# caomuqing/neptune

Measured on AMD Instinct MI355X. Metric: backend_replans_per_sec, higher is better.
Workload: dtype f64; 1 GPU; 64 agents + 20 static obstacles, K=8, 128 seeded scenes in flight per GPU per step (seeds 0..127 over 1 GPU); the handle's default solve path: verified line presolve 4 m, polish on; agents=64, obstacles=20, scenes_per_gpu=128, scenes_in_flight=128, scene_groups=1

## Files before the change

### include/neptune_backend_debug.h

```cpp
#ifndef NEPTUNE_BACKEND_DEBUG_H
#define NEPTUNE_BACKEND_DEBUG_H

#include "neptune_backend.h"

#ifdef __cplusplus
extern "C" {
#endif

int nep_backend_debug_time_sequence(nep_backend_t* h, const nep_pwp* init, int32_t n_obst, const int32_t* hull_off,
                                    const double* hull_xy, const int32_t* h0_off, const double* h0_xy, const nep_ent_view* ent,
                                    double t_start, double dc, int32_t n_iter, double* us_out, double* us_optimize_out);

int nep_backend_debug_set_lines(nep_backend_t* h, int32_t n_lines, const int32_t* seg,
                                const double* nd);
int nep_backend_debug_get_lines(nep_backend_t* h, int32_t cap, int32_t* seg, double* nd,
                                int32_t* n_out);

int nep_debug_regroup_records(const nep_traj_rec* d_src, nep_traj_rec* d_dst, int32_t world, int32_t n_scenes,
                              int32_t n_local, void* stream);

int nep_batch_debug_redo_count(nep_batch_t* h, int32_t* by_reason);
int nep_batch_debug_redo_list(nep_batch_t* h, int32_t* slots_out, int32_t cap);

int64_t nep_batch_line_bucket_bytes(nep_batch_t* h);
// ... 16 lines not shown

int nep_batch_debug_conflicts(nep_batch_t* h, int32_t scene, uint8_t* conflict_out);
int nep_batch_debug_conflicts_prev(nep_batch_t* h, int32_t scene, uint8_t* conflict_out);

int nep_batch_kernel_time(nep_batch_t* h, int32_t which, double* avg_ms, int32_t* n_launch);
int nep_batch_enable_timing(nep_batch_t* h, int32_t on);
int nep_batch_reset_timing(nep_batch_t* h);

enum {
  NEP_PATH_BOX_KERNEL = 1,
  NEP_PATH_HULLS_GROUPED = 2,
  NEP_PATH_FUSED_BOXES = 4,
  NEP_PATH_FUSED_ORDER = 8,
  NEP_PATH_ORDERED_QP = 16,
  NEP_PATH_PRESOLVE_KERNEL = 32,
  NEP_PATH_REDO_PASS = 64
};
int nep_batch_debug_launch_path(nep_batch_t* h, int32_t* bits);
int nep_batch_debug_boxes(nep_batch_t* h, int32_t scene, double* out, int32_t cap);
int nep_batch_debug_order_keys(nep_batch_t* h, int32_t* keys, int32_t cap);

int nep_batch_debug_hulls(nep_batch_t* h, int32_t scene, double* hull_xy, int32_t* hull_nv);
int nep_batch_debug_lines(nep_batch_t* h, int32_t slot, int32_t cap, int32_t* seg, double* nd,
                          int32_t* n_out);

int nep_batch_debug_phase_cycles(nep_batch_t* h, int32_t slot, int64_t* out16);

int nep_batch_fe_search_us(nep_batch_t* h, float* us, int32_t cap);

int nep_batch_set_fe_ent_fast_caps(nep_batch_t* h, int32_t list_cap, int32_t add_cap, int32_t bend_cap);

// ... 10 lines not shown
```

### neptune_amd/abi.py

```python
import ctypes as C

import numpy as np

NEP_MAX_POL = 8
NEP_TRAJ_MAX_SEG = 16
NEP_HULL_MAX_V = 16
NEP_HULL_MAX_CP = 16
NEP_MAX_BEND = 8
NEP_STATE_DOUBLES = 12

NEP_OK, NEP_RELAXED, NEP_FAILED = 0, 1, 2
NEP_SKIPPED = 3
NEP_FE_SKIPPED = 4


class nep_pwp(C.Structure):
    _fields_ = [("n_seg", C.c_int32), ("_pad", C.c_int32),
                ("times", C.c_double * (NEP_TRAJ_MAX_SEG + 1)),
                ("coeff", ((C.c_double * 4) * NEP_TRAJ_MAX_SEG) * 3)]


class nep_traj_rec(C.Structure):
    _fields_ = [("id", C.c_int32), ("is_agent", C.c_int32), ("n_bend", C.c_int32),
                ("valid", C.c_int32),
                ("bbox", C.c_double * 3), ("pos", C.c_double * 3),
                ("bend", (C.c_double * 2) * NEP_MAX_BEND),
                ("pwp", nep_pwp)]

# ... 187 lines not shown
```

### neptune_amd/backend.py

```python
import ctypes as C

import numpy as np

from . import abi
from ._lib import BackendError, check, lib


def _csr(polys):
    off = np.zeros(len(polys) + 1, dtype=np.int32)
    for k, p in enumerate(polys):
        off[k + 1] = off[k] + len(p)
    xy = (np.concatenate([np.asarray(p, dtype=np.float64).reshape(-1, 2) for p in polys])
          if len(polys) and off[-1] > 0 else np.zeros((0, 2)))
    return off, np.ascontiguousarray(xy, dtype=np.float64)


def make_pwp(times, coeff):
    p = abi.nep_pwp()
    K = coeff.shape[1]
    p.n_seg = K
    for i in range(K + 1):
        p.times[i] = float(times[i])
    arr = np.ctypeslib.as_array(p.coeff)
    arr[:, :K, :] = coeff
# ... 426 lines not shown
    def qp_kernel_name(self):
        return "qp_reg_kernel" if lib().nep_batch_qp_placement(self._h) == 1 else "qp_kernel"

    def set_hull_kernel(self, mode=0):
        check(lib().nep_batch_set_hull_kernel(self._h, int(mode)))

    def set_launch_order(self, enable=True):
        check(lib().nep_batch_set_launch_order(self._h, 1 if enable else 0))

    def launch_order(self):
        out = np.zeros(self.n_scenes * self.n_local, dtype=np.int32); n = C.c_int32(0)
        check(lib().nep_batch_debug_launch_order(self._h, abi.iptr(out), len(out), C.byref(n)))
        return out[:n.value].copy() if n.value else None

    LAUNCH_PATH = (("box_kernel", 1), ("grouped_hulls", 2), ("fused_boxes", 4), ("fused_order", 8), ("ordered_qp", 16),
                   ("presolve_kernel", 32), ("redo_pass", 64))

    def debug_launch_path(self):
        b = C.c_int32(0)
        check(lib().nep_batch_debug_launch_path(self._h, C.byref(b)))
        return {name: bool(b.value & bit) for name, bit in self.LAUNCH_PATH}

    def debug_boxes(self, scene=0):
        out = np.zeros((self.N + self.n_static, self.par.num_pol, 4))
        check(lib().nep_batch_debug_boxes(self._h, int(scene), abi.dptr(out), out.size))
        return out

    def debug_order_keys(self):
        out = np.zeros(self.slots, dtype=np.int32)
        check(lib().nep_batch_debug_order_keys(self._h, abi.iptr(out), len(out)))
        return out
# ... 129 lines not shown
```

### neptune_amd/csrc/backend.hip

```cpp
#include <hip/hip_runtime.h>

#include <atomic>
#include <chrono>
#include <cmath>
#include <cstdio>
#include <cstdlib>
#include <cstring>
#include <memory>
#include <string>
#include <vector>

#include "nep_device.h"
#include "audit_common.h"
#include "mission_common.h"
#include "../../include/neptune_plan.h"
#include "../../include/neptune_entangle.h"

using namespace nep;

namespace nep { DebugGlobals g_debug; }

namespace {

thread_local std::string g_err;
// ... 343 lines not shown
  }
  hipEvent_t next_event() {
    if (ev_used == ev.size()) { hipEvent_t e; hipEventCreate(&e); ev.push_back(e); }
    return ev[ev_used++];
  }
  int run(const nep_traj_rec* d_recs, int n_rec, ProblemSet& ps, hipStream_t st, int phases = 3) {
    const int slots = n_scenes * sp.n_local;
    SampleSched sc{d_sched_n.p, d_sched_seg.p, d_sched_dt.p};
    const bool geo = (phases & 1) != 0, qp = (phases & 2) != 0;
    if (timing) hipEventRecord(next_event(), st);
    const bool fused_boxes = d_recs && geo && ps.skip_box != nullptr && !ps.lines_override && static_boxes_ok && ps.hull_pb <= 0
                             && n_rec == sp.num_agents && sp.n_hull == sp.num_agents && hulls_grouped(sp, n_scenes, n_rec);
    const bool want_order = qp && lpt && have_history && slots > 1024 && d_order_key.n >= (size_t)slots && d_order.n >= (size_t)slots;
    const bool fused_order = fused_boxes && want_order;
    if (fused_order) { ps.order = d_order.p; ps.order_key = d_order_key.p; }
    if (geo) last_path = 0; else last_path &= NEP_PATH_BOX_KERNEL | NEP_PATH_HULLS_GROUPED | NEP_PATH_FUSED_BOXES | NEP_PATH_FUSED_ORDER;
    if (d_recs && geo) launch_hulls(d_recs, n_scenes, n_rec, ps.guess, sp, ps, st, fused_boxes);
    if (d_recs && geo && hulls_grouped(sp, n_scenes, n_rec)) last_path |= NEP_PATH_HULLS_GROUPED;
    if (fused_boxes) last_path |= NEP_PATH_FUSED_BOXES;
    if (fused_order) last_path |= NEP_PATH_FUSED_ORDER;
    if (timing) hipEventRecord(next_event(), st);
    if (ps.lines_override) { ps.skip_box = nullptr; ps.line_skip = nullptr; ps.redo_list = nullptr; ps.redo_count = nullptr; }
    if (scratch_chunks > 0 && ps.scratch_chunks == 0) {
      scratch_full = true;
      HIPCHK(hipStreamSynchronize(st));
      if (int e = size_row_scratch()) return e;
      ps.row_scratch = d_row_scratch.p;
    }
    const bool skip = ps.skip_box != nullptr;
    if (!ps.lines_override && geo) {
      if (skip && !fused_boxes) { launch_boxes(n_scenes, sp, ps, st); last_path |= NEP_PATH_BOX_KERNEL; }
      launch_separator(slots, sp, ps, st);
    }
// ... 1378 lines not shown
  return 0;
}
int nep_batch_debug_set_option(nep_batch_t* h, const char* name, int32_t value) { if (!h) return fail(NEP_E_ARG, "null handle"); return engine_option(h->eng, name, value); }
int nep_backend_debug_set_option(nep_backend_t* h, const char* name, int32_t value) { if (!h) return fail(NEP_E_ARG, "null handle"); return engine_option(h->eng, name, value); }
int nep_debug_set_global_option(const char* name, int32_t value) {
  if (!name) return fail(NEP_E_ARG, "null option name");
  const std::string n(name);
  if (n == "fe_three") g_debug.fe_three = value != 0;
  else if (n == "fe_xcd") g_debug.fe_xcd = value;
  else if (n == "polish_grid") { if (value < 1) return fail(NEP_E_ARG, "polish_grid >= 1"); g_debug.polish_grid = value; }
  else return fail(NEP_E_ARG, "unknown global debug option: " + n);
  return 0;
}

int nep_batch_set_hull_kernel(nep_batch_t* h, int32_t mode) {
  if (!h || mode < 0 || mode > 2) return fail(NEP_E_ARG, "mode: 0 automatic, 1 one hull per wave, 2 eight hulls per wave");
  h->eng.sp.hull_mode = mode;
  return 0;
}

int nep_batch_set_max_runtime(nep_batch_t* h, double seconds) {
  if (!h || !(seconds >= 0.0)) return fail(NEP_E_ARG, "bad arguments");
  h->eng.sp.time_limit_ticks = seconds > 0 ? (long long)(seconds * h->eng.clock_hz) : 0;
  return 0;
}

namespace {
int set_line_cull(Engine* E, double radius) {
  if (!E || !(radius >= 0.0)) return fail(NEP_E_ARG, "bad arguments");
  E->sp.cull_radius = radius; E->cull_user_set = true;
  return 0;
// ... 206 lines not shown
```

### neptune_amd/csrc/geom_kernels.hip

```cpp
#include <hip/hip_runtime.h>

#include <cstdlib>
#include <cstring>

#include "nep_device.h"
#include "../../include/neptune_frontend.h"
#include "ent_device.h"

namespace nep {

__constant__ double cAPosInv[4][4] = {
    {-0.03203276669713047, -0.09273093424558249, 0.3420572455666699, 1.1023313949144335},
    {-0.05111494245568798, -0.046272612998418894, 0.5458234872124772, 1.0979806946005568},
    {-0.07454781852812224, 0.203951949894552, 0.796048050105448, 1.0745478185281223},
    {1.0, 1.0, 0.9999999999999996, 0.9999999999999993}};

#define SEP_MIN_GAP 1e-7
#define NEP_INF (__builtin_huge_val())

__device__ __forceinline__ double cross3(double ox, double oy, double ax, double ay, double bx, double by) {
  return (ax - ox) * (by - oy) - (ay - oy) * (bx - ox);
}
__device__ __forceinline__ bool lex_less(double ax, double ay, double bx, double by) {
  return ax < bx || (ax == bx && ay < by);
// ... 165 lines not shown
      const bool m_lt = (kx[r] < ox) | ((kx[r] == ox) & (ky[r] < oy));
      const bool take = want_min ? o_lt : m_lt;
      kx[r] = take ? ox : kx[r]; ky[r] = take ? oy : ky[r];
    }
  }
}
template <int J, int K_, int JJ> __device__ __forceinline__ void grp_bitonic_merge(double (&kx)[J], double (&ky)[J], int sub) {
  grp_bitonic_step<J, K_, JJ>(kx, ky, sub);
  if constexpr (JJ > 1) grp_bitonic_merge<J, K_, JJ / 2>(kx, ky, sub);
}
template <int J, int K_> __device__ __forceinline__ void grp_bitonic(double (&kx)[J], double (&ky)[J], int sub) {
  if constexpr (K_ > 2) grp_bitonic<J, K_ / 2>(kx, ky, sub);
  grp_bitonic_merge<J, K_, K_ / 2>(kx, ky, sub);
}

template <int J>
__device__ __forceinline__ int group_hull(int n, const double (&px)[J], const double (&py)[J], double* sxy, int g, int sub,
                                          bool write, double* __restrict__ out_xy, int cap) {
  constexpr int kGrpPts = J;
  __syncthreads();
  {
    double kx[J], ky[J];
#pragma unroll
    for (int j = 0; j < J; j++) { const bool in = sub + 8 * j < n; kx[j] = in ? px[j] : NEP_INF; ky[j] = in ? py[j] : NEP_INF; }
    grp_bitonic<J, 8 * J>(kx, ky, sub);
#pragma unroll
    for (int r = 0; r < J; r++) { const int e = sub * J + r; if (e < n) { sxy[2 * e] = kx[r]; sxy[2 * e + 1] = ky[r]; } }
  }
  __syncthreads();
  double ux[kGrpPts], uy[kGrpPts]; int pos[kGrpPts]; bool keep[kGrpPts];
  int m = 0;
#pragma unroll
  for (int j = 0; j < kGrpPts; j++) {
    const int p = sub + 8 * j;
    ux[j] = 0; uy[j] = 0; keep[j] = false;
    if (p < n) { ux[j] = sxy[2 * p]; uy[j] = sxy[2 * p + 1]; keep[j] = p == 0 || ux[j] != sxy[2 * p - 2] || uy[j] != sxy[2 * p - 1]; }
    const unsigned bits = (unsigned)(__ballot(keep[j]) >> (8 * g)) & 0xffu;
    pos[j] = m + __popc(bits & ((1u << sub) - 1u));
    m += __popc(bits);
  }
  __syncthreads();
#pragma unroll
  for (int j = 0; j < kGrpPts; j++) { if (keep[j]) { sxy[2 * pos[j]] = ux[j]; sxy[2 * pos[j] + 1] = uy[j]; } }
  __syncthreads();
  unsigned long long mask = 0;
  if (sub < 2 && m >= 2) {
    const bool lower = sub == 0;
    int kc = 0;
    int i1 = 0, i2 = 0;
    double ax = 0, ay = 0, bx = 0, by = 0;
    for (int i = 0; i < m; i++) {
      const double2 c = *(const double2*)(sxy + 2 * (lower ? i : m - 1 - i));
      const double x = c.x, y = c.y;
      while (kc >= 2 && cross3(ax, ay, bx, by, x, y) <= 0.0) {
        mask &= ~(1ull << i1);
        kc--; bx = ax; by = ay; i1 = i2;
        if (kc >= 2) {
          i2 = 63 - __clzll((long long)(mask & ((1ull << i2) - 1ull)));
          const double2 a = *(const double2*)(sxy + 2 * (lower ? i2 : m - 1 - i2));
          ax = a.x; ay = a.y;
        }
      }
      mask |= 1ull << i; kc++;
      ax = bx; ay = by; bx = x; by = y;
      i2 = i1; i1 = i;
    }
  }
  const unsigned long long L = __shfl(mask, 8 * g), U = __shfl(mask, 8 * g + 1);
  const int kl = __popcll(L), ku = __popcll(U);
  const int k = m >= 2 ? kl + ku - 2 : m;
  if (write) {
    if (m == 1) { if (sub == 0 && cap > 0) { out_xy[0] = sxy[0]; out_xy[1] = sxy[1]; } }
    else if (m >= 2) {
#pragma unroll
      for (int j = 0; j < kGrpPts; j++) {
        const int p = sub + 8 * j;
        if (p < m) {
          const double x = sxy[2 * p], y = sxy[2 * p + 1];
          if ((L >> p) & 1ull) { const int o = __popcll(L & ((1ull << p) - 1ull)); if (o < cap) { out_xy[2 * o] = x; out_xy[2 * o + 1] = y; } }
          const int iu = m - 1 - p;
          if (((U >> iu) & 1ull) && p != 0 && p != m - 1) {
            const int o = kl + __popcll(U & ((1ull << iu) - 1ull)) - 1;
            if (o < cap) { out_xy[2 * o] = x; out_xy[2 * o + 1] = y; }
          }
        }
      }
    }
  }
  return k;
}

__global__ __launch_bounds__(64) void hull_group_kernel(const nep_traj_rec* __restrict__ recs, int n_rec_per_scene,
                                                        const double* __restrict__ ts0, long ts_scene_stride,
                                                        int num_pol, double T_span, double drone_radius,
                                                        double* __restrict__ hull_xy, int* __restrict__ hull_nv,
                                                        double* __restrict__ hull0_xy, int* __restrict__ hull0_nv,
                                                        double* __restrict__ bend_xy, int* __restrict__ bend_n, int* __restrict__ flags,
                                                        double* __restrict__ box_out, int box_per_scene, int* __restrict__ zero4,
                                                        int n_traj, int ord_n, const int* __restrict__ ord_key, int* __restrict__ ord_out, int* __restrict__ ord_zero4) {
  __shared__ __attribute__((aligned(16))) double s_sxy[8][kGrpSxy];
  __shared__ double s_cpx[8][kHullCP], s_cpy[8][kHullCP];
  double* stimes = &s_sxy[7][0];
  static_assert(NEP_TRAJ_MAX_SEG + 2 <= kGrpSxy, "the knot vector borrows a group's point area");
  const int lane = threadIdx.x, g = lane >> 3, sub = lane & 7;
  if (ord_n > 0 && blockIdx.x == 0) {
    if (ord_zero4 && lane < 4) ord_zero4[lane] = 0;
    int* hist = (int*)&s_sxy[0][0];
    int* tot = hist + 64 * 16;
    for (int i = lane; i < 64 * 16; i += 64) hist[i] = 0;
    __syncthreads();
    const int su = lane & 15;
    for (int i0 = 0; i0 < ord_n; i0 += 1024) {
      int kk[16];
#pragma unroll
      for (int u = 0; u < 16; u++) { const int i = i0 + 64 * u + lane; kk[u] = i < ord_n ? ord_key[i] : 0; }
#pragma unroll
      for (int u = 0; u < 16; u++) { const int i = i0 + 64 * u + lane; if (i < ord_n) atomicAdd(&hist[(63 - (kk[u] & 63)) * 16 + su], 1); }
    }
    __syncthreads();
    { int o = 0; for (int u = 0; u < 16; u++) { const int c = hist[lane * 16 + u]; hist[lane * 16 + u] = o; o += c; } tot[lane] = o; }
    __syncthreads();
    if (lane == 0) { int o = 0; for (int b = 0; b < 64; b++) { const int c = tot[b]; tot[b] = o; o += c; } }
    __syncthreads();
    for (int i0 = 0; i0 < ord_n; i0 += 1024) {
      int kk[16];
#pragma unroll
      for (int u = 0; u < 16; u++) { const int i = i0 + 64 * u + lane; kk[u] = i < ord_n ? ord_key[i] : 0; }
#pragma unroll
      for (int u = 0; u < 16; u++) { const int i = i0 + 64 * u + lane; if (i < ord_n) { const int b = 63 - (kk[u] & 63); ord_out[tot[b] + atomicAdd(&hist[b * 16 + su], 1)] = i; } }
    }
    return;
  }
  const int jt = (int)blockIdx.x - (ord_n > 0 ? 1 : 0);
  const int scene = jt / n_rec_per_scene;
  const nep_traj_rec* r = recs + jt;
  if (lane == 0 && bend_n) {
    int nb = r->n_bend; if (nb > kBend) nb = kBend; if (nb < 0) nb = 0;
    bend_n[jt] = (r->valid && r->is_agent) ? nb : 0;
    for (int b = 0; b < nb; b++) { bend_xy[((long)jt * kBend + b) * 2] = r->bend[b][0]; bend_xy[((long)jt * kBend + b) * 2 + 1] = r->bend[b][1]; }
  }
  const bool act = g < num_pol;
  const long out = (long)jt * num_pol + g;
  if (zero4 && jt == 0 && lane < 4) zero4[lane] = 0;
  double* box = box_out ? box_out + (((long)scene * box_per_scene + (jt - scene * n_rec_per_scene)) * num_pol + g) * 4 : nullptr;
  if (!(r->valid && r->is_agent) || r->pwp.n_seg <= 0) {
    if (act && sub == 0) { hull_nv[out] = 0; if (hull0_nv) hull0_nv[out] = 0; if (box) { box[0] = NEP_INF; box[1] = -NEP_INF; box[2] = NEP_INF; box[3] = -NEP_INF; } }
    return;
  }
  const double ts = *(const double*)((const char*)ts0 + (long)scene * ts_scene_stride);
  const double t0 = ts + g * T_span, t1 = ts + (g + 1) * T_span;
  const int n = r->pwp.n_seg;
  if (lane <= n) stimes[lane] = r->pwp.times[lane];
  __syncthreads();
  int first = -1, last = -1;
  for (int k = 0; k <= n; k++) { const double tk = stimes[k]; first += tk < t0 ? 1 : 0; last += tk <= t1 ? 1 : 0; }
  if (first < 0) first = 0; if (first > n - 1) first = n - 1;
  if (last < 0) last = 0; if (last > n - 1) last = n - 1;
  int nseg = last - first + 1; if (nseg < 0) nseg = 0;
  if (nseg > kHullCP / 4) { nseg = kHullCP / 4; if (act && sub == 0 && flags) atomicOr(flags, NEP_FLAG_HULL_OVERFLOW); }
  if (!act) nseg = 0;
  const int np0 = 4 * nseg;
  double* cpx = s_cpx[g]; double* cpy = s_cpy[g];
  for (int v = sub; v < 2 * np0; v += 8) {
    const int sl = v >> 3, k = (v >> 1) & 3, ax = v & 1;
    const int s = first + sl;
    double _t;
    if (s != last) _t = stimes[s + 1] - stimes[s];
    else if (t1 > stimes[s + 1]) _t = stimes[s + 1] - stimes[s];
    else _t = t1 - stimes[s];
    if (_t > T_span) _t = T_span; else if (_t < 0) _t = 0;
    const double c0 = _t * _t * _t, c1 = _t * _t, c2 = _t, c3 = 1.0;
    const double* P = r->pwp.coeff[ax][s];
    const double val = (((P[0] * c0) * cAPosInv[0][k] + (P[1] * c1) * cAPosInv[1][k]) + (P[2] * c2) * cAPosInv[2][k]) + (P[3] * c3) * cAPosInv[3][k];
    if (ax == 0) cpx[sl * 4 + k] = val; else cpy[sl * 4 + k] = val;
  }
  __syncthreads();
  const double dx = r->bbox[0] / 2.0 + drone_radius, dy = r->bbox[1] / 2.0 + drone_radius;
  const bool inflate = !(sqrt(dx * dx + dy * dy) < 1e-6);
  const int np = inflate ? 4 * np0 : np0;
  double px[kGrpPts], py[kGrpPts];
#pragma unroll
  for (int j = 0; j < kGrpPts; j++) {
    const int p = sub + 8 * j;
    px[j] = 0; py[j] = 0;
    if (p < np) {
      if (inflate) {
        const int c = p >> 2, q = p & 3;
        const double x = cpx[c], y = cpy[c];
        px[j] = (q < 2) ? x + dx : x - dx;
        py[j] = (q == 0 || q == 3) ? y + dy : y - dy;
      } else { px[j] = cpx[p]; py[j] = cpy[p]; }
    }
  }
  if (box) {
    double x0 = NEP_INF, x1 = -NEP_INF, y0 = NEP_INF, y1 = -NEP_INF;
#pragma unroll
    for (int j = 0; j < 2; j++) { const int p = sub + 8 * j; if (p < np0) { const double x = cpx[p], y = cpy[p]; x0 = fmin(x0, x); x1 = fmax(x1, x); y0 = fmin(y0, y); y1 = fmax(y1, y); } }
    auto shl4 = [](double v) { return __hiloint2double(__builtin_amdgcn_mov_dpp(__double2hiint(v), 0x104, 0xf, 0xf, false), __builtin_amdgcn_mov_dpp(__double2loint(v), 0x104, 0xf, 0xf, false)); };
    x0 = fmin(x0, shl4(x0)); x1 = fmax(x1, shl4(x1)); y0 = fmin(y0, shl4(y0)); y1 = fmax(y1, shl4(y1));
    x0 = fmin(x0, grp_xor<2>(x0)); x1 = fmax(x1, grp_xor<2>(x1)); y0 = fmin(y0, grp_xor<2>(y0)); y1 = fmax(y1, grp_xor<2>(y1));
    x0 = fmin(x0, grp_xor<1>(x0)); x1 = fmax(x1, grp_xor<1>(x1)); y0 = fmin(y0, grp_xor<1>(y0)); y1 = fmax(y1, grp_xor<1>(y1));
    if (act && sub == 0) {
      if (np0 <= 0) { box[0] = NEP_INF; box[1] = -NEP_INF; box[2] = NEP_INF; box[3] = -NEP_INF; }
      else if (inflate) { box[0] = x0 - dx; box[1] = x1 + dx; box[2] = y0 - dy; box[3] = y1 + dy; }
      else { box[0] = x0; box[1] = x1; box[2] = y0; box[3] = y1; }
    }
  }
  int k = group_hull<kGrpPts>(np, px, py, s_sxy[g], g, sub, act, hull_xy + out * kHullV * 2, kHullV);
  if (k > kHullV) { k = kHullV; if (act && sub == 0 && flags) atomicOr(flags, NEP_FLAG_HULL_OVERFLOW); }
  if (act && sub == 0) hull_nv[out] = k;
  if (hull0_nv) {
    double qx[2], qy[2];
#pragma unroll
    for (int j = 0; j < 2; j++) { const int p = sub + 8 * j; qx[j] = p < np0 ? cpx[p] : 0; qy[j] = p < np0 ? cpy[p] : 0; }
    int k0 = group_hull<2>(np0, qx, qy, s_sxy[g], g, sub, act, hull0_xy + out * 2, 1);
    if (k0 > kHullV) k0 = kHullV;
    if (act && sub == 0) hull0_nv[out] = k0;
  }
}

bool hulls_grouped(const SceneParams& sp, int n_scenes, int n_rec) {
  return sp.num_pol <= 8 && (sp.hull_mode ? sp.hull_mode == 2 : (long)n_scenes * n_rec > 2048);
}
void launch_hulls(const nep_traj_rec* recs, int n_scenes, int n_rec, const nep_guess* guess,
                  const SceneParams& sp, const ProblemSet& ps, hipStream_t st, bool boxes) {
  launch_hulls_ts(recs, n_scenes, n_rec, &guess->t_start, (long)sizeof(nep_guess), sp, ps, st, boxes);
}
void launch_hulls_ts(const nep_traj_rec* recs, int n_scenes, int n_rec, const double* ts0, long ts_slot_stride,
                     const SceneParams& sp, const ProblemSet& ps, hipStream_t st, bool boxes) {
  int blocks = n_scenes * n_rec * sp.num_pol;
  if (blocks <= 0) return;
  const bool need0 = sp.ent_enabled != 0;
  const bool grouped = sp.hull_mode ? sp.hull_mode == 2 : (long)n_scenes * n_rec > 2048;
  if (sp.num_pol <= 8 && grouped) {
    const bool ord = boxes && ps.order != nullptr && ps.order_key != nullptr;
    hipLaunchKernelGGL(hull_group_kernel, dim3(n_scenes * n_rec + (ord ? 1 : 0)), dim3(64), 0, st, recs, n_rec, ts0, ts_slot_stride * sp.n_local,
                       sp.num_pol, sp.T_span, sp.drone_radius, ps.hull_xy, ps.hull_nv, need0 ? ps.hull0_xy : nullptr,
                       need0 ? ps.hull0_nv : nullptr, need0 ? ps.bend_xy : nullptr, need0 ? ps.bend_n : nullptr, ps.flags,
                       boxes ? ps.fe_box : nullptr, sp.num_agents + sp.n_static, boxes ? ps.redo_count : nullptr,
                       n_scenes * n_rec, ord ? n_scenes * sp.n_local : 0, ord ? (const int*)ps.order_key : nullptr, ord ? (int*)ps.order : nullptr, ord ? ps.polish_count : nullptr);
    return;
  }
  hipLaunchKernelGGL(hull_kernel, dim3(blocks), dim3(64), 0, st, recs, n_rec, ts0, ts_slot_stride * sp.n_local,
                     sp.num_pol, sp.T_span, sp.drone_radius, ps.hull_xy, ps.hull_nv, need0 ? ps.hull0_xy : nullptr,
                     need0 ? ps.hull0_nv : nullptr, need0 ? ps.bend_xy : nullptr, need0 ? ps.bend_n : nullptr, ps.flags);
}

struct SepBest { bool have; double num, len2, tA, nx, ny, px, py; };

__device__ __forceinline__ void sep_consider(SepBest& b, double num, double len2, double tA, double nx, double ny, double px, double py) {
  const bool better = (num > 0.0) & ((num * num) * b.len2 > (b.num * b.num) * len2);
  if (better) { b.have = true; b.num = num; b.len2 = len2; b.tA = tA; b.nx = nx; b.ny = ny; b.px = px; b.py = py; }
}

struct Pts4 { double x[4], y[4]; };
// ... 1172 lines not shown
  __syncthreads();
  const int words = (int)(sizeof(nep_traj_rec) / sizeof(double));
  for (long e = (long)part * blockDim.x + tid; e < (long)N * words; e += (long)blockDim.x * kResolveParts) {
    const int a = (int)(e / words), w = (int)(e % words);
    const double* src = (const double*)((sAcc[a] ? fresh : prev) + (long)scene * N + a);
    ((double*)(final_out + (long)scene * N + a))[w] = src[w];
  }
  if (accept_out && part == 0) for (int a = tid; a < N; a += blockDim.x) accept_out[(long)scene * N + a] = sAcc[a];
}

void launch_safety(const nep_traj_rec* prev, const nep_traj_rec* fresh, int n_scenes, int N, const SceneParams& sp, const ProblemSet& ps,
                   unsigned char* conflict, unsigned char* conflict_prev, const int* entangles, nep_traj_rec* final_out, int* accept_out, hipStream_t st,
                   const int* active) {
  if (n_scenes * N <= 0) return;
  auto hulls_of = [&](const nep_traj_rec* recs) {
    if (sp.num_pol <= 8 && (sp.hull_mode ? sp.hull_mode == 2 : (long)n_scenes * N > 2048))
      hipLaunchKernelGGL(hull_group_kernel, dim3(n_scenes * N), dim3(64), 0, st, recs, N, &ps.guess->t_start, (long)sizeof(nep_guess) * sp.n_local, sp.num_pol, sp.T_span,
                         sp.drone_radius, ps.hull_xy, ps.hull_nv, (double*)nullptr, (int*)nullptr, (double*)nullptr, (int*)nullptr, ps.flags,
                         (double*)nullptr, 0, (int*)nullptr, n_scenes * N, 0, (const int*)nullptr, (int*)nullptr, (int*)nullptr);
    else
      hipLaunchKernelGGL(hull_kernel, dim3(n_scenes * N * sp.num_pol), dim3(64), 0, st, recs, N, &ps.guess->t_start, (long)sizeof(nep_guess) * sp.n_local, sp.num_pol, sp.T_span,
                         sp.drone_radius, ps.hull_xy, ps.hull_nv, (double*)nullptr, (int*)nullptr, (double*)nullptr, (int*)nullptr, ps.flags);
  };
  if (conflict_prev) {
    hulls_of(prev);
    hipLaunchKernelGGL(safety_conflict_kernel, dim3(n_scenes * ((N + 3) / 4)), dim3(256), 0, st, fresh, prev, N, sp.num_pol, sp.T_span, ps.hull_xy, ps.hull_nv, conflict_prev);
  }
  hulls_of(fresh);
  hipLaunchKernelGGL(safety_conflict_kernel, dim3(n_scenes * ((N + 3) / 4)), dim3(256), 0, st, fresh, fresh, N, sp.num_pol, sp.T_span, ps.hull_xy, ps.hull_nv, conflict);
  const size_t resolve_lds = (size_t)(2 * N + (N + 1) * ((N + 31) / 32)) * sizeof(int);
  static DynLdsAttr resolve_attr;
  (void)resolve_attr.ensure((const void*)safety_resolve_kernel, resolve_lds);
  hipLaunchKernelGGL(safety_resolve_kernel, dim3(n_scenes * kResolveParts), dim3(256), resolve_lds, st, prev, fresh, N, conflict, conflict_prev, entangles, final_out, accept_out, active);
}
// ... 1120 lines not shown
```

### neptune_amd/csrc/nep_device.h

```cpp
#pragma once
#include <hip/hip_runtime.h>

#include <mutex>

#include "nep_tables.h"
#include "../../include/neptune_frontend.h"
#include "../../include/neptune_fleet.h"
#include "../../include/neptune_backend_debug.h"

namespace nep {

constexpr int kHullV = NEP_HULL_MAX_V;
constexpr int kHullCP = NEP_HULL_MAX_CP;
constexpr int kBend = NEP_MAX_BEND;

struct DebugGlobals { bool fe_three = false; int fe_xcd = 1; int polish_grid = 256; };
extern DebugGlobals g_debug;

constexpr int kCorrFromItDefault = 10, kCorrMaxCountDefault = 8;
struct SceneParams {
  int num_agents;
  int num_pol;
  int n_static;
  int n_hull;
// ... 99 lines not shown
    std::lock_guard<std::mutex> lk(mu);
    if (bytes <= configured[dev]) return hipSuccess;
    const hipError_t e = hipFuncSetAttribute(fn, hipFuncAttributeMaxDynamicSharedMemorySize, (int)bytes);
    if (e == hipSuccess) configured[dev] = bytes;
    return e;
  }
};

struct SampleSched {
  const int* n;
  const int* seg;
  const double* dt;
};

bool hulls_grouped(const SceneParams& sp, int n_scenes, int n_rec);
void launch_hulls(const nep_traj_rec* recs, int n_scenes, int n_rec, const nep_guess* guess,
                  const SceneParams& sp, const ProblemSet& ps, hipStream_t st, bool boxes = false);
void launch_hulls_ts(const nep_traj_rec* recs, int n_scenes, int n_rec, const double* ts0, long ts_slot_stride,
                     const SceneParams& sp, const ProblemSet& ps, hipStream_t st, bool boxes = false);
void launch_hulls_explicit(const nep_traj_rec* recs, int n_traj, double t_start, int num_pol,
                           double T_span, double drone_radius, double* hull_xy, int* hull_nv,
                           double* hull0_xy, int* hull0_nv, int* flags, hipStream_t st);
void launch_separator(int n_slots, const SceneParams& sp, const ProblemSet& ps, hipStream_t st);
void launch_separator_redo(int n_slots, const SceneParams& sp, const ProblemSet& ps, hipStream_t st);
void launch_boxes(int n_scenes, const SceneParams& sp, const ProblemSet& ps, hipStream_t st);
void launch_active_rows(int n_slots, const SceneParams& sp, const ProblemSet& ps, double tol, int* out, hipStream_t st);
void launch_separator_explicit(int n_prob, const int* a_off, const double* a_xy, const int* b_off,
                               const double* b_xy, double* nd, int* solved, int rule, hipStream_t st);
void launch_qp(int n_slots, const SceneParams& sp, const ProblemSet& ps, const QpTable* tables,
               const SampleSched& sched, size_t lds_bytes, hipStream_t st);
// ... 139 lines not shown
```

Measured before the change: 20.85 million replans/s.

## Add four-trajectory-per-workgroup hull kernel with wave-level sync for large batches

Adds a hull_quad_kernel that packs four trajectories into one 256-thread workgroup, one wave each. It replaces workgroup barriers with wave-local fence and barrier builtins, and spreads the monotone-chain step across the waves. The old grouped kernel is split into reusable helpers (sort/unique, chain, write, point generation, order histogram) shared by both kernels. The new kernel is chosen automatically when the trajectory count exceeds 4096, which the default 128-scene, 64-agent config does. The aim is fewer, fuller workgroups and cheaper synchronization, at the cost of more shared memory per workgroup and more code complexity.

```diff
diff --git a/include/neptune_backend_debug.h b/include/neptune_backend_debug.h
--- a/include/neptune_backend_debug.h
+++ b/include/neptune_backend_debug.h
@@ -54,7 +54,8 @@
   NEP_PATH_FUSED_ORDER = 8,
   NEP_PATH_ORDERED_QP = 16,
   NEP_PATH_PRESOLVE_KERNEL = 32,
-  NEP_PATH_REDO_PASS = 64
+  NEP_PATH_REDO_PASS = 64,
+  NEP_PATH_HULLS_QUAD = 128
 };
 int nep_batch_debug_launch_path(nep_batch_t* h, int32_t* bits);
 int nep_batch_debug_boxes(nep_batch_t* h, int32_t scene, double* out, int32_t cap);
diff --git a/neptune_amd/abi.py b/neptune_amd/abi.py
--- a/neptune_amd/abi.py
+++ b/neptune_amd/abi.py
@@ -12,6 +12,7 @@
 NEP_OK, NEP_RELAXED, NEP_FAILED = 0, 1, 2
 NEP_SKIPPED = 3
 NEP_FE_SKIPPED = 4
+NEP_PATH_HULLS_QUAD = 128
 
 
 class nep_pwp(C.Structure):
diff --git a/neptune_amd/backend.py b/neptune_amd/backend.py
--- a/neptune_amd/backend.py
+++ b/neptune_amd/backend.py
@@ -464,7 +464,7 @@
         return out[:n.value].copy() if n.value else None
 
     LAUNCH_PATH = (("box_kernel", 1), ("grouped_hulls", 2), ("fused_boxes", 4), ("fused_order", 8), ("ordered_qp", 16),
-                   ("presolve_kernel", 32), ("redo_pass", 64))
+                   ("presolve_kernel", 32), ("redo_pass", 64), ("quad_hulls", abi.NEP_PATH_HULLS_QUAD))
 
     def debug_launch_path(self):
         b = C.c_int32(0)
diff --git a/neptune_amd/csrc/backend.hip b/neptune_amd/csrc/backend.hip
--- a/neptune_amd/csrc/backend.hip
+++ b/neptune_amd/csrc/backend.hip
@@ -381,9 +381,10 @@
     const bool want_order = qp && lpt && have_history && slots > 1024 && d_order_key.n >= (size_t)slots && d_order.n >= (size_t)slots;
     const bool fused_order = fused_boxes && want_order;
     if (fused_order) { ps.order = d_order.p; ps.order_key = d_order_key.p; }
-    if (geo) last_path = 0; else last_path &= NEP_PATH_BOX_KERNEL | NEP_PATH_HULLS_GROUPED | NEP_PATH_FUSED_BOXES | NEP_PATH_FUSED_ORDER;
+    if (geo) last_path = 0; else last_path &= NEP_PATH_BOX_KERNEL | NEP_PATH_HULLS_GROUPED | NEP_PATH_HULLS_QUAD | NEP_PATH_FUSED_BOXES | NEP_PATH_FUSED_ORDER;
     if (d_recs && geo) launch_hulls(d_recs, n_scenes, n_rec, ps.guess, sp, ps, st, fused_boxes);
     if (d_recs && geo && hulls_grouped(sp, n_scenes, n_rec)) last_path |= NEP_PATH_HULLS_GROUPED;
+    if (d_recs && geo && hulls_quad(sp, n_scenes, n_rec)) last_path |= NEP_PATH_HULLS_QUAD;
     if (fused_boxes) last_path |= NEP_PATH_FUSED_BOXES;
     if (fused_order) last_path |= NEP_PATH_FUSED_ORDER;
     if (timing) hipEventRecord(next_event(), st);
@@ -1792,7 +1793,7 @@
 }
 
 int nep_batch_set_hull_kernel(nep_batch_t* h, int32_t mode) {
-  if (!h || mode < 0 || mode > 2) return fail(NEP_E_ARG, "mode: 0 automatic, 1 one hull per wave, 2 eight hulls per wave");
+  if (!h || mode < 0 || mode > 3) return fail(NEP_E_ARG, "mode: 0 automatic, 1 one hull per wave, 2 eight hulls per wave, 3 four trajectories per workgroup");
   h->eng.sp.hull_mode = mode;
   return 0;
 }
diff --git a/neptune_amd/csrc/geom_kernels.hip b/neptune_amd/csrc/geom_kernels.hip
--- a/neptune_amd/csrc/geom_kernels.hip
+++ b/neptune_amd/csrc/geom_kernels.hip
@@ -203,11 +203,15 @@
   grp_bitonic_merge<J, K_, K_ / 2>(kx, ky, sub);
 }
 
-template <int J>
-__device__ __forceinline__ int group_hull(int n, const double (&px)[J], const double (&py)[J], double* sxy, int g, int sub,
-                                          bool write, double* __restrict__ out_xy, int cap) {
+template <bool WaveSync> __device__ __forceinline__ void grp_sync() {
+  if constexpr (WaveSync) { __builtin_amdgcn_fence(__ATOMIC_RELEASE, "workgroup"); __builtin_amdgcn_wave_barrier(); __builtin_amdgcn_fence(__ATOMIC_ACQUIRE, "workgroup"); }
+  else __syncthreads();
+}
+
+template <int J, bool WaveSync>
+__device__ __forceinline__ int grp_sort_unique(int n, const double (&px)[J], const double (&py)[J], double* sxy, int g, int sub) {
   constexpr int kGrpPts = J;
-  __syncthreads();
+  grp_sync<WaveSync>();
   {
     double kx[J], ky[J];
 #pragma unroll
@@ -216,7 +220,7 @@
 #pragma unroll
     for (int r = 0; r < J; r++) { const int e = sub * J + r; if (e < n) { sxy[2 * e] = kx[r]; sxy[2 * e + 1] = ky[r]; } }
   }
-  __syncthreads();
+  grp_sync<WaveSync>();
   double ux[kGrpPts], uy[kGrpPts]; int pos[kGrpPts]; bool keep[kGrpPts];
   int m = 0;
 #pragma unroll
@@ -228,34 +232,41 @@
     pos[j] = m + __popc(bits & ((1u << sub) - 1u));
     m += __popc(bits);
   }
-  __syncthreads();
+  grp_sync<WaveSync>();
 #pragma unroll
   for (int j = 0; j < kGrpPts; j++) { if (keep[j]) { sxy[2 * pos[j]] = ux[j]; sxy[2 * pos[j] + 1] = uy[j]; } }
-  __syncthreads();
+  grp_sync<WaveSync>();
+  return m;
+}
+
+__device__ __forceinline__ unsigned long long grp_chain(const double* sxy, int m, bool lower) {
   unsigned long long mask = 0;
-  if (sub < 2 && m >= 2) {
-    const bool lower = sub == 0;
-    int kc = 0;
-    int i1 = 0, i2 = 0;
-    double ax = 0, ay = 0, bx = 0, by = 0;
-    for (int i = 0; i < m; i++) {
-      const double2 c = *(const double2*)(sxy + 2 * (lower ? i : m - 1 - i));
-      const double x = c.x, y = c.y;
-      while (kc >= 2 && cross3(ax, ay, bx, by, x, y) <= 0.0) {
-        mask &= ~(1ull << i1);
-        kc--; bx = ax; by = ay; i1 = i2;
-        if (kc >= 2) {
-          i2 = 63 - __clzll((long long)(mask & ((1ull << i2) - 1ull)));
-          const double2 a = *(const double2*)(sxy + 2 * (lower ? i2 : m - 1 - i2));
-          ax = a.x; ay = a.y;
-        }
-      }
-      mask |= 1ull << i; kc++;
-      ax = bx; ay = by; bx = x; by = y;
-      i2 = i1; i1 = i;
-    }
-  }
-  const unsigned long long L = __shfl(mask, 8 * g), U = __shfl(mask, 8 * g + 1);
+  int kc = 0;
+  int i1 = 0, i2 = 0;
+  double ax = 0, ay = 0, bx = 0, by = 0;
+  for (int i = 0; i < m; i++) {
+    const double2 c = *(const double2*)(sxy + 2 * (lower ? i : m - 1 - i));
+    const double x = c.x, y = c.y;
+    while (kc >= 2 && cross3(ax, ay, bx, by, x, y) <= 0.0) {
+      mask &= ~(1ull << i1);
+      kc--; bx = ax; by = ay; i1 = i2;
+      if (kc >= 2) {
+        i2 = 63 - __clzll((long long)(mask & ((1ull << i2) - 1ull)));
+        const double2 a = *(const double2*)(sxy + 2 * (lower ? i2 : m - 1 - i2));
+        ax = a.x; ay = a.y;
+      }
+    }
+    mask |= 1ull << i; kc++;
+    ax = bx; ay = by; bx = x; by = y;
+    i2 = i1; i1 = i;
+  }
+  return mask;
+}
+
+template <int J>
+__device__ __forceinline__ int grp_write(int m, unsigned long long L, unsigned long long U, const double* sxy, int sub,
+                                         bool write, double* __restrict__ out_xy, int cap) {
+  constexpr int kGrpPts = J;
   const int kl = __popcll(L), ku = __popcll(U);
   const int k = m >= 2 ? kl + ku - 2 : m;
   if (write) {
@@ -279,6 +290,106 @@
   return k;
 }
 
+template <int J>
+__device__ __forceinline__ int group_hull(int n, const double (&px)[J], const double (&py)[J], double* sxy, int g, int sub,
+                                          bool write, double* __restrict__ out_xy, int cap) {
+  const int m = grp_sort_unique<J, false>(n, px, py, sxy, g, sub);
+  unsigned long long mask = 0;
+  if (sub < 2 && m >= 2) mask = grp_chain(sxy, m, sub == 0);
+  const unsigned long long L = __shfl(mask, 8 * g), U = __shfl(mask, 8 * g + 1);
+  return grp_write<J>(m, L, U, sxy, sub, write, out_xy, cap);
+}
+
+template <bool WaveSync>
+__device__ __forceinline__ void order_block(int lane, int* hist, int ord_n, const int* __restrict__ ord_key, int* __restrict__ ord_out, int* __restrict__ ord_zero4) {
+  if (ord_zero4 && lane < 4) ord_zero4[lane] = 0;
+  int* tot = hist + 64 * 16;
+  for (int i = lane; i < 64 * 16; i += 64) hist[i] = 0;
+  grp_sync<WaveSync>();
+  const int su = lane & 15;
+  for (int i0 = 0; i0 < ord_n; i0 += 1024) {
+    int kk[16];
+#pragma unroll
+    for (int u = 0; u < 16; u++) { const int i = i0 + 64 * u + lane; kk[u] = i < ord_n ? ord_key[i] : 0; }
+#pragma unroll
+    for (int u = 0; u < 16; u++) { const int i = i0 + 64 * u + lane; if (i < ord_n) atomicAdd(&hist[(63 - (kk[u] & 63)) * 16 + su], 1); }
+  }
+  grp_sync<WaveSync>();
+  { int o = 0; for (int u = 0; u < 16; u++) { const int c = hist[lane * 16 + u]; hist[lane * 16 + u] = o; o += c; } tot[lane] = o; }
+  grp_sync<WaveSync>();
+  if (lane == 0) { int o = 0; for (int b = 0; b < 64; b++) { const int c = tot[b]; tot[b] = o; o += c; } }
+  grp_sync<WaveSync>();
+  for (int i0 = 0; i0 < ord_n; i0 += 1024) {
+    int kk[16];
+#pragma unroll
+    for (int u = 0; u < 16; u++) { const int i = i0 + 64 * u + lane; kk[u] = i < ord_n ? ord_key[i] : 0; }
+#pragma unroll
+    for (int u = 0; u < 16; u++) { const int i = i0 + 64 * u + lane; if (i < ord_n) { const int b = 63 - (kk[u] & 63); ord_out[tot[b] + atomicAdd(&hist[b * 16 + su], 1)] = i; } }
+  }
+}
+
+template <bool WaveSync>
+__device__ __forceinline__ void grp_points(const nep_traj_rec* __restrict__ r, double ts, int g, int sub, bool act, double T_span, double drone_radius,
+                                           double* stimes, double* cpx, double* cpy, int* __restrict__ flags, double* __restrict__ box,
+                                           int& np, int& np0, double (&px)[kGrpPts], double (&py)[kGrpPts]) {
+  const double t0 = ts + g * T_span, t1 = ts + (g + 1) * T_span;
+  const int n = r->pwp.n_seg;
+  const int lane = 8 * g + sub;
+  if (lane <= n) stimes[lane] = r->pwp.times[lane];
+  grp_sync<WaveSync>();
+  int first = -1, last = -1;
+  for (int k = 0; k <= n; k++) { const double tk = stimes[k]; first += tk < t0 ? 1 : 0; last += tk <= t1 ? 1 : 0; }
+  if (first < 0) first = 0; if (first > n - 1) first = n - 1;
+  if (last < 0) last = 0; if (last > n - 1) last = n - 1;
+  int nseg = last - first + 1; if (nseg < 0) nseg = 0;
+  if (nseg > kHullCP / 4) { nseg = kHullCP / 4; if (act && sub == 0 && flags) atomicOr(flags, NEP_FLAG_HULL_OVERFLOW); }
+  if (!act) nseg = 0;
+  np0 = 4 * nseg;
+  for (int v = sub; v < 2 * np0; v += 8) {
+    const int sl = v >> 3, k = (v >> 1) & 3, ax = v & 1;
+    const int s = first + sl;
+    double _t;
+    if (s != last) _t = stimes[s + 1] - stimes[s];
+    else if (t1 > stimes[s + 1]) _t = stimes[s + 1] - stimes[s];
+    else _t = t1 - stimes[s];
+    if (_t > T_span) _t = T_span; else if (_t < 0) _t = 0;
+    const double c0 = _t * _t * _t, c1 = _t * _t, c2 = _t, c3 = 1.0;
+    const double* P = r->pwp.coeff[ax][s];
+    const double val = (((P[0] * c0) * cAPosInv[0][k] + (P[1] * c1) * cAPosInv[1][k]) + (P[2] * c2) * cAPosInv[2][k]) + (P[3] * c3) * cAPosInv[3][k];
+    if (ax == 0) cpx[sl * 4 + k] = val; else cpy[sl * 4 + k] = val;
+  }
+  grp_sync<WaveSync>();
+  const double dx = r->bbox[0] / 2.0 + drone_radius, dy = r->bbox[1] / 2.0 + drone_radius;
+  const bool inflate = !(sqrt(dx * dx + dy * dy) < 1e-6);
+  np = inflate ? 4 * np0 : np0;
+#pragma unroll
+  for (int j = 0; j < kGrpPts; j++) {
+    const int p = sub + 8 * j;
+    px[j] = 0; py[j] = 0;
+    if (p < np) {
+      if (inflate) {
+        const int c = p >> 2, q = p & 3;
+        const double x = cpx[c], y = cpy[c];
+        px[j] = (q < 2) ? x + dx : x - dx;
+        py[j] = (q == 0 || q == 3) ? y + dy : y - dy;
+      } else { px[j] = cpx[p]; py[j] = cpy[p]; }
+    }
+  }
+  if (box) {
+    double x0 = NEP_INF, x1 = -NEP_INF, y0 = NEP_INF, y1 = -NEP_INF;
+#pragma unroll
+    for (int j = 0; j < 2; j++) { const int p = sub + 8 * j; if (p < np0) { const double x = cpx[p], y = cpy[p]; x0 = fmin(x0, x); x1 = fmax(x1, x); y0 = fmin(y0, y); y1 = fmax(y1, y); } }
+    auto shl4 = [](double v) { return __hiloint2double(__builtin_amdgcn_mov_dpp(__double2hiint(v), 0x104, 0xf, 0xf, false), __builtin_amdgcn_mov_dpp(__double2loint(v), 0x104, 0xf, 0xf, false)); };
+    x0 = fmin(x0, shl4(x0)); x1 = fmax(x1, shl4(x1)); y0 = fmin(y0, shl4(y0)); y1 = fmax(y1, shl4(y1));
+    x0 = fmin(x0, grp_xor<2>(x0)); x1 = fmax(x1, grp_xor<2>(x1)); y0 = fmin(y0, grp_xor<2>(y0)); y1 = fmax(y1, grp_xor<2>(y1));
+    x0 = fmin(x0, grp_xor<1>(x0)); x1 = fmax(x1, grp_xor<1>(x1)); y0 = fmin(y0, grp_xor<1>(y0)); y1 = fmax(y1, grp_xor<1>(y1));
+    if (act && sub == 0) {
+      if (np0 <= 0) { box[0] = NEP_INF; box[1] = -NEP_INF; box[2] = NEP_INF; box[3] = -NEP_INF; }
+      else if (inflate) { box[0] = x0 - dx; box[1] = x1 + dx; box[2] = y0 - dy; box[3] = y1 + dy; }
+      else { box[0] = x0; box[1] = x1; box[2] = y0; box[3] = y1; }
+    }
+  }
+}
 __global__ __launch_bounds__(64) void hull_group_kernel(const nep_traj_rec* __restrict__ recs, int n_rec_per_scene,
                                                         const double* __restrict__ ts0, long ts_scene_stride,
                                                         int num_pol, double T_span, double drone_radius,
@@ -293,31 +404,7 @@
   static_assert(NEP_TRAJ_MAX_SEG + 2 <= kGrpSxy, "the knot vector borrows a group's point area");
   const int lane = threadIdx.x, g = lane >> 3, sub = lane & 7;
   if (ord_n > 0 && blockIdx.x == 0) {
-    if (ord_zero4 && lane < 4) ord_zero4[lane] = 0;
-    int* hist = (int*)&s_sxy[0][0];
-    int* tot = hist + 64 * 16;
-    for (int i = lane; i < 64 * 16; i += 64) hist[i] = 0;
-    __syncthreads();
-    const int su = lane & 15;
-    for (int i0 = 0; i0 < ord_n; i0 += 1024) {
-      int kk[16];
-#pragma unroll
-      for (int u = 0; u < 16; u++) { const int i = i0 + 64 * u + lane; kk[u] = i < ord_n ? ord_key[i] : 0; }
-#pragma unroll
-      for (int u = 0; u < 16; u++) { const int i = i0 + 64 * u + lane; if (i < ord_n) atomicAdd(&hist[(63 - (kk[u] & 63)) * 16 + su], 1); }
-    }
-    __syncthreads();
-    { int o = 0; for (int u = 0; u < 16; u++) { const int c = hist[lane * 16 + u]; hist[lane * 16 + u] = o; o += c; } tot[lane] = o; }
-    __syncthreads();
-    if (lane == 0) { int o = 0; for (int b = 0; b < 64; b++) { const int c = tot[b]; tot[b] = o; o += c; } }
-    __syncthreads();
-    for (int i0 = 0; i0 < ord_n; i0 += 1024) {
-      int kk[16];
-#pragma unroll
-      for (int u = 0; u < 16; u++) { const int i = i0 + 64 * u + lane; kk[u] = i < ord_n ? ord_key[i] : 0; }
-#pragma unroll
-      for (int u = 0; u < 16; u++) { const int i = i0 + 64 * u + lane; if (i < ord_n) { const int b = 63 - (kk[u] & 63); ord_out[tot[b] + atomicAdd(&hist[b * 16 + su], 1)] = i; } }
-    }
+    order_block<false>(lane, (int*)&s_sxy[0][0], ord_n, ord_key, ord_out, ord_zero4);
     return;
   }
   const int jt = (int)blockIdx.x - (ord_n > 0 ? 1 : 0);
@@ -337,64 +424,10 @@
     return;
   }
   const double ts = *(const double*)((const char*)ts0 + (long)scene * ts_scene_stride);
-  const double t0 = ts + g * T_span, t1 = ts + (g + 1) * T_span;
-  const int n = r->pwp.n_seg;
-  if (lane <= n) stimes[lane] = r->pwp.times[lane];
-  __syncthreads();
-  int first = -1, last = -1;
-  for (int k = 0; k <= n; k++) { const double tk = stimes[k]; first += tk < t0 ? 1 : 0; last += tk <= t1 ? 1 : 0; }
-  if (first < 0) first = 0; if (first > n - 1) first = n - 1;
-  if (last < 0) last = 0; if (last > n - 1) last = n - 1;
-  int nseg = last - first + 1; if (nseg < 0) nseg = 0;
-  if (nseg > kHullCP / 4) { nseg = kHullCP / 4; if (act && sub == 0 && flags) atomicOr(flags, NEP_FLAG_HULL_OVERFLOW); }
-  if (!act) nseg = 0;
-  const int np0 = 4 * nseg;
   double* cpx = s_cpx[g]; double* cpy = s_cpy[g];
-  for (int v = sub; v < 2 * np0; v += 8) {
-    const int sl = v >> 3, k = (v >> 1) & 3, ax = v & 1;
-    const int s = first + sl;
-    double _t;
-    if (s != last) _t = stimes[s + 1] - stimes[s];
-    else if (t1 > stimes[s + 1]) _t = stimes[s + 1] - stimes[s];
-    else _t = t1 - stimes[s];
-    if (_t > T_span) _t = T_span; else if (_t < 0) _t = 0;
-    const double c0 = _t * _t * _t, c1 = _t * _t, c2 = _t, c3 = 1.0;
-    const double* P = r->pwp.coeff[ax][s];
-    const double val = (((P[0] * c0) * cAPosInv[0][k] + (P[1] * c1) * cAPosInv[1][k]) + (P[2] * c2) * cAPosInv[2][k]) + (P[3] * c3) * cAPosInv[3][k];
-    if (ax == 0) cpx[sl * 4 + k] = val; else cpy[sl * 4 + k] = val;
-  }
-  __syncthreads();
-  const double dx = r->bbox[0] / 2.0 + drone_radius, dy = r->bbox[1] / 2.0 + drone_radius;
-  const bool inflate = !(sqrt(dx * dx + dy * dy) < 1e-6);
-  const int np = inflate ? 4 * np0 : np0;
+  int np, np0;
   double px[kGrpPts], py[kGrpPts];
-#pragma unroll
-  for (int j = 0; j < kGrpPts; j++) {
-    const int p = sub + 8 * j;
-    px[j] = 0; py[j] = 0;
-    if (p < np) {
-      if (inflate) {
-        const int c = p >> 2, q = p & 3;
-        const double x = cpx[c], y = cpy[c];
-        px[j] = (q < 2) ? x + dx : x - dx;
-        py[j] = (q == 0 || q == 3) ? y + dy : y - dy;
-      } else { px[j] = cpx[p]; py[j] = cpy[p]; }
-    }
-  }
-  if (box) {
-    double x0 = NEP_INF, x1 = -NEP_INF, y0 = NEP_INF, y1 = -NEP_INF;
-#pragma unroll
-    for (int j = 0; j < 2; j++) { const int p = sub + 8 * j; if (p < np0) { const double x = cpx[p], y = cpy[p]; x0 = fmin(x0, x); x1 = fmax(x1, x); y0 = fmin(y0, y); y1 = fmax(y1, y); } }
-    auto shl4 = [](double v) { return __hiloint2double(__builtin_amdgcn_mov_dpp(__double2hiint(v), 0x104, 0xf, 0xf, false), __builtin_amdgcn_mov_dpp(__double2loint(v), 0x104, 0xf, 0xf, false)); };
-    x0 = fmin(x0, shl4(x0)); x1 = fmax(x1, shl4(x1)); y0 = fmin(y0, shl4(y0)); y1 = fmax(y1, shl4(y1));
-    x0 = fmin(x0, grp_xor<2>(x0)); x1 = fmax(x1, grp_xor<2>(x1)); y0 = fmin(y0, grp_xor<2>(y0)); y1 = fmax(y1, grp_xor<2>(y1));
-    x0 = fmin(x0, grp_xor<1>(x0)); x1 = fmax(x1, grp_xor<1>(x1)); y0 = fmin(y0, grp_xor<1>(y0)); y1 = fmax(y1, grp_xor<1>(y1));
-    if (act && sub == 0) {
-      if (np0 <= 0) { box[0] = NEP_INF; box[1] = -NEP_INF; box[2] = NEP_INF; box[3] = -NEP_INF; }
-      else if (inflate) { box[0] = x0 - dx; box[1] = x1 + dx; box[2] = y0 - dy; box[3] = y1 + dy; }
-      else { box[0] = x0; box[1] = x1; box[2] = y0; box[3] = y1; }
-    }
-  }
+  grp_points<false>(r, ts, g, sub, act, T_span, drone_radius, stimes, cpx, cpy, flags, box, np, np0, px, py);
   int k = group_hull<kGrpPts>(np, px, py, s_sxy[g], g, sub, act, hull_xy + out * kHullV * 2, kHullV);
   if (k > kHullV) { k = kHullV; if (act && sub == 0 && flags) atomicOr(flags, NEP_FLAG_HULL_OVERFLOW); }
   if (act && sub == 0) hull_nv[out] = k;
@@ -408,9 +441,95 @@
   }
 }
 
-bool hulls_grouped(const SceneParams& sp, int n_scenes, int n_rec) {
-  return sp.num_pol <= 8 && (sp.hull_mode ? sp.hull_mode == 2 : (long)n_scenes * n_rec > 2048);
-}
+constexpr int kQuadCp = 2 * 8 * kHullCP;
+static_assert(kQuadCp >= 16 + 4, "the 16 masks and the 8 point counts of a wave borrow its control-point area");
+static_assert(sizeof(double) * (8 * kGrpSxy + kQuadCp) == 10240, "a wave's LDS is exactly 10 KB: sixteen waves per CU, as in hull_group_kernel");
+
+template <int J>
+__device__ __forceinline__ int quad_hull(bool live, int n, const double (&px)[J], const double (&py)[J], double (*s_sxy)[8][kGrpSxy], double (*s_cp)[kQuadCp],
+                                         int wv, int lane, bool chain_wave, bool write, double* __restrict__ out_xy, int cap) {
+  const int g = lane >> 3, sub = lane & 7;
+  double* sxy = s_sxy[wv][g];
+  const int m = live ? grp_sort_unique<J, true>(n, px, py, sxy, g, sub) : 0;
+  if (sub == 0) ((int*)(s_cp[wv] + 16))[g] = m;
+  __syncthreads();
+  if (chain_wave) {
+    const int cw = lane >> 4, cg = (lane >> 1) & 7;
+    const int cm = ((const int*)(s_cp[cw] + 16))[cg];
+    unsigned long long mask = 0;
+    if (cm >= 2) mask = grp_chain(s_sxy[cw][cg], cm, (lane & 1) == 0);
+    ((unsigned long long*)s_cp[cw])[lane & 15] = mask;
+  }
+  __syncthreads();
+  const unsigned long long* s_mask = (const unsigned long long*)s_cp[wv];
+  return grp_write<J>(m, s_mask[2 * g], s_mask[2 * g + 1], sxy, sub, write, out_xy, cap);
+}
+
+__global__ __launch_bounds__(256, 4) void hull_quad_kernel(const nep_traj_rec* __restrict__ recs, int n_rec_per_scene,
+                                                           const double* __restrict__ ts0, long ts_scene_stride,
+                                                           int num_pol, double T_span, double drone_radius,
+                                                           double* __restrict__ hull_xy, int* __restrict__ hull_nv,
+                                                           double* __restrict__ hull0_xy, int* __restrict__ hull0_nv,
+                                                           double* __restrict__ bend_xy, int* __restrict__ bend_n, int* __restrict__ flags,
+                                                           double* __restrict__ box_out, int box_per_scene, int* __restrict__ zero4,
+                                                           int n_traj, int ord_n, const int* __restrict__ ord_key, int* __restrict__ ord_out, int* __restrict__ ord_zero4) {
+  __shared__ __attribute__((aligned(16))) double s_sxy[4][8][kGrpSxy];
+  __shared__ __attribute__((aligned(16))) double s_cp[4][kQuadCp];
+  static_assert(sizeof(double) * 4 * (8 * kGrpSxy + kQuadCp) <= 40960, "four workgroups per CU");
+  const int wv = __builtin_amdgcn_readfirstlane(threadIdx.x >> 6), lane = threadIdx.x & 63, g = lane >> 3, sub = lane & 7;
+  if (ord_n > 0 && blockIdx.x == 0) {
+    if (wv == 0) order_block<true>(lane, (int*)&s_sxy[0][0][0], ord_n, ord_key, ord_out, ord_zero4);
+    return;
+  }
+  const int blk = (int)blockIdx.x - (ord_n > 0 ? 1 : 0);
+  const int jt = 4 * blk + wv;
+  const bool in = jt < n_traj;
+  const nep_traj_rec* r = recs + (in ? jt : 0);
+  const int scene = (in ? jt : 0) / n_rec_per_scene;
+  if (in && lane == 0 && bend_n) {
+    int nb = r->n_bend; if (nb > kBend) nb = kBend; if (nb < 0) nb = 0;
+    bend_n[jt] = (r->valid && r->is_agent) ? nb : 0;
+    for (int b = 0; b < nb; b++) { bend_xy[((long)jt * kBend + b) * 2] = r->bend[b][0]; bend_xy[((long)jt * kBend + b) * 2 + 1] = r->bend[b][1]; }
+  }
+  const long out = (long)jt * num_pol + g;
+  if (zero4 && jt == 0 && lane < 4) zero4[lane] = 0;
+  double* box = box_out && in ? box_out + (((long)scene * box_per_scene + (jt - scene * n_rec_per_scene)) * num_pol + g) * 4 : nullptr;
+  const bool live = __builtin_amdgcn_readfirstlane(in && r->valid && r->is_agent && r->pwp.n_seg > 0 ? 1 : 0) != 0;
+  if (in && !live && g < num_pol && sub == 0) {
+    hull_nv[out] = 0; if (hull0_nv) hull0_nv[out] = 0;
+    if (box) { box[0] = NEP_INF; box[1] = -NEP_INF; box[2] = NEP_INF; box[3] = -NEP_INF; }
+  }
+  const bool act = live && g < num_pol;
+  double* cpx = s_cp[wv] + g * kHullCP; double* cpy = s_cp[wv] + (8 + g) * kHullCP;
+  int np = 0, np0 = 0;
+  double px[kGrpPts], py[kGrpPts], qx[2] = {0, 0}, qy[2] = {0, 0};
+  if (live) {
+    const double ts = *(const double*)((const char*)ts0 + (long)scene * ts_scene_stride);
+    grp_points<true>(r, ts, g, sub, act, T_span, drone_radius, &s_sxy[wv][7][0], cpx, cpy, flags, box, np, np0, px, py);
+    if (hull0_nv) {
+#pragma unroll
+      for (int j = 0; j < 2; j++) { const int p = sub + 8 * j; qx[j] = p < np0 ? cpx[p] : 0; qy[j] = p < np0 ? cpy[p] : 0; }
+    }
+  }
+  const bool chain_wave = wv == (blk & 3);
+  int k = quad_hull<kGrpPts>(live, np, px, py, s_sxy, s_cp, wv, lane, chain_wave, act, hull_xy + out * kHullV * 2, kHullV);
+  if (k > kHullV) { k = kHullV; if (act && sub == 0 && flags) atomicOr(flags, NEP_FLAG_HULL_OVERFLOW); }
+  if (act && sub == 0) hull_nv[out] = k;
+  if (hull0_nv) {
+    int k0 = quad_hull<2>(live, np0, qx, qy, s_sxy, s_cp, wv, lane, chain_wave, act, hull0_xy + out * 2, 1);
+    if (k0 > kHullV) k0 = kHullV;
+    if (act && sub == 0) hull0_nv[out] = k0;
+  }
+}
+
+constexpr long kQuadMin = 4096;
+static int hull_kernel_of(const SceneParams& sp, long n_traj) {
+  if (sp.num_pol > 8) return 1;
+  if (sp.hull_mode) return sp.hull_mode;
+  return n_traj > kQuadMin ? 3 : n_traj > 2048 ? 2 : 1;
+}
+bool hulls_grouped(const SceneParams& sp, int n_scenes, int n_rec) { return hull_kernel_of(sp, (long)n_scenes * n_rec) >= 2; }
+bool hulls_quad(const SceneParams& sp, int n_scenes, int n_rec) { return hull_kernel_of(sp, (long)n_scenes * n_rec) == 3; }
 void launch_hulls(const nep_traj_rec* recs, int n_scenes, int n_rec, const nep_guess* guess,
                   const SceneParams& sp, const ProblemSet& ps, hipStream_t st, bool boxes) {
   launch_hulls_ts(recs, n_scenes, n_rec, &guess->t_start, (long)sizeof(nep_guess), sp, ps, st, boxes);
@@ -420,14 +539,18 @@
   int blocks = n_scenes * n_rec * sp.num_pol;
   if (blocks <= 0) return;
   const bool need0 = sp.ent_enabled != 0;
-  const bool grouped = sp.hull_mode ? sp.hull_mode == 2 : (long)n_scenes * n_rec > 2048;
-  if (sp.num_pol <= 8 && grouped) {
+  const int kern = hull_kernel_of(sp, (long)n_scenes * n_rec);
+  if (kern >= 2) {
     const bool ord = boxes && ps.order != nullptr && ps.order_key != nullptr;
-    hipLaunchKernelGGL(hull_group_kernel, dim3(n_scenes * n_rec + (ord ? 1 : 0)), dim3(64), 0, st, recs, n_rec, ts0, ts_slot_stride * sp.n_local,
-                       sp.num_pol, sp.T_span, sp.drone_radius, ps.hull_xy, ps.hull_nv, need0 ? ps.hull0_xy : nullptr,
-                       need0 ? ps.hull0_nv : nullptr, need0 ? ps.bend_xy : nullptr, need0 ? ps.bend_n : nullptr, ps.flags,
-                       boxes ? ps.fe_box : nullptr, sp.num_agents + sp.n_static, boxes ? ps.redo_count : nullptr,
-                       n_scenes * n_rec, ord ? n_scenes * sp.n_local : 0, ord ? (const int*)ps.order_key : nullptr, ord ? (int*)ps.order : nullptr, ord ? ps.polish_count : nullptr);
+    const int n_traj = n_scenes * n_rec;
+    auto go = [&](auto kernel, int n_blocks, int threads) {
+      hipLaunchKernelGGL(kernel, dim3(n_blocks + (ord ? 1 : 0)), dim3(threads), 0, st, recs, n_rec, ts0, ts_slot_stride * sp.n_local,
+                         sp.num_pol, sp.T_span, sp.drone_radius, ps.hull_xy, ps.hull_nv, need0 ? ps.hull0_xy : nullptr,
+                         need0 ? ps.hull0_nv : nullptr, need0 ? ps.bend_xy : nullptr, need0 ? ps.bend_n : nullptr, ps.flags,
+                         boxes ? ps.fe_box : nullptr, sp.num_agents + sp.n_static, boxes ? ps.redo_count : nullptr,
+                         n_traj, ord ? n_scenes * sp.n_local : 0, ord ? (const int*)ps.order_key : nullptr, ord ? (int*)ps.order : nullptr, ord ? ps.polish_count : nullptr);
+    };
+    if (kern == 3) go(hull_quad_kernel, (n_traj + 3) / 4, 256); else go(hull_group_kernel, n_traj, 64);
     return;
   }
   hipLaunchKernelGGL(hull_kernel, dim3(blocks), dim3(64), 0, st, recs, n_rec, ts0, ts_slot_stride * sp.n_local,
@@ -1630,10 +1753,14 @@
                    const int* active) {
   if (n_scenes * N <= 0) return;
   auto hulls_of = [&](const nep_traj_rec* recs) {
-    if (sp.num_pol <= 8 && (sp.hull_mode ? sp.hull_mode == 2 : (long)n_scenes * N > 2048))
-      hipLaunchKernelGGL(hull_group_kernel, dim3(n_scenes * N), dim3(64), 0, st, recs, N, &ps.guess->t_start, (long)sizeof(nep_guess) * sp.n_local, sp.num_pol, sp.T_span,
+    const int kern = hull_kernel_of(sp, (long)n_scenes * N);
+    auto go = [&](auto kernel, int n_blocks, int threads) {
+      hipLaunchKernelGGL(kernel, dim3(n_blocks), dim3(threads), 0, st, recs, N, &ps.guess->t_start, (long)sizeof(nep_guess) * sp.n_local, sp.num_pol, sp.T_span,
                          sp.drone_radius, ps.hull_xy, ps.hull_nv, (double*)nullptr, (int*)nullptr, (double*)nullptr, (int*)nullptr, ps.flags,
                          (double*)nullptr, 0, (int*)nullptr, n_scenes * N, 0, (const int*)nullptr, (int*)nullptr, (int*)nullptr);
+    };
+    if (kern == 3) go(hull_quad_kernel, (n_scenes * N + 3) / 4, 256);
+    else if (kern == 2) go(hull_group_kernel, n_scenes * N, 64);
     else
       hipLaunchKernelGGL(hull_kernel, dim3(n_scenes * N * sp.num_pol), dim3(64), 0, st, recs, N, &ps.guess->t_start, (long)sizeof(nep_guess) * sp.n_local, sp.num_pol, sp.T_span,
                          sp.drone_radius, ps.hull_xy, ps.hull_nv, (double*)nullptr, (int*)nullptr, (double*)nullptr, (int*)nullptr, ps.flags);
diff --git a/neptune_amd/csrc/nep_device.h b/neptune_amd/csrc/nep_device.h
--- a/neptune_amd/csrc/nep_device.h
+++ b/neptune_amd/csrc/nep_device.h
@@ -137,6 +137,7 @@
 };
 
 bool hulls_grouped(const SceneParams& sp, int n_scenes, int n_rec);
+bool hulls_quad(const SceneParams& sp, int n_scenes, int n_rec);
 void launch_hulls(const nep_traj_rec* recs, int n_scenes, int n_rec, const nep_guess* guess,
                   const SceneParams& sp, const ProblemSet& ps, hipStream_t st, bool boxes = false);
 void launch_hulls_ts(const nep_traj_rec* recs, int n_scenes, int n_rec, const double* ts0, long ts_slot_stride,
```

New measurement: 21.05 million replans/s, median of 6. Within noise of the previous version (+1.0%).
